# tomwhite/disq

Measured on AMD Instinct MI355X. Metric: decompressed BAM GB/s + reads/sec (whole node) at 1/2/4/8 MI355X, higher is better.
Workload: dtype u8

## Files before the change

### disq_amd/csrc/dq_api.hip

```cpp
#include <hip/hip_runtime.h>

#include <fcntl.h>
#include <sys/stat.h>
#include <unistd.h>

#include <algorithm>
#include <chrono>
#include <cstdio>
#include <cstdlib>
#include <cstring>
#include <map>
#include <string>
#include <thread>
#include <type_traits>
#include <sys/mman.h>
#include <mutex>
#include <vector>

#include "../../include/disq_gpu.h"
#include "dq_internal.h"
#include "dq_sam_core.h"
#include "dq_vcf_core.h"
#include "dq_vcf_gt_core.h"
#include "dq_vcf_info_core.h"
// ... 647 lines not shown
  }
  dbg(s, "chain", nblk, broken);
  ctx->nblk = nblk;
  if (nblk == 0 && L > 0) RET(DQ_EFORMAT, "no BGZF blocks found");
  ctx->ulen = ulen;
  HIPCHK(hipEventRecord(ctx->ev[1], s));
  if ((rc = ensure_all(ctx, ctx->U, (size_t)ulen + 256))) return rc;
  if ((rc = ensure_all(ctx, ctx->status, sizeof(int32_t) * (size_t)(nblk + 1)))) return rc;
  HIPCHK(hipMemsetAsync(ctx->status.p, 0, sizeof(int32_t) * (size_t)(nblk + 1), s));
  HIPCHK(hipMemsetAsync(ctx->U.as<uint8_t>() + ulen, 0, 256, s));
  {
    const uint32_t* crc_init = inflate3_tables(ctx->o.device);
    if (!crc_init) RET(DQ_EDEVICE, "CRC32 table initialisation failed on this device");
    static const bool timing = getenv("DQ_TIMING") != nullptr;
    uint64_t* tim = nullptr;
    if (timing) {
      HIPCHK(hipMalloc(&tim, sizeof(uint64_t) * INFLATE_TIM_WORDS * (size_t)std::max<int64_t>(1, nblk)));
      HIPCHK(hipMemsetAsync(tim, 0, sizeof(uint64_t) * INFLATE_TIM_WORDS * (size_t)std::max<int64_t>(1, nblk), s));
    }
    HIPCHK(hipEventRecord(ctx->ev[5], s));
    if ((rc = ensure_all(ctx, ctx->tails, INFLATE_SCRATCH_BYTES * (size_t)std::max<int64_t>(1, nblk)))) return rc;
    launch_inflate3(ctx->cbuf(), ctx->blk_pos.as<int64_t>(), ctx->blk_cs.as<int32_t>(),
                    ctx->blk_us.as<int32_t>(), ctx->uoff.as<int64_t>(), nblk, ctx->U.as<uint8_t>(),
                    ctx->status.as<int32_t>(), ctx->o.verify_crc, crc_init, tim, s, nullptr, 0,
                    ctx->tails.p);
    HIPCHK(hipEventRecord(ctx->ev[6], s));
    if (timing) {
      std::vector<uint64_t> h(INFLATE_TIM_WORDS * (size_t)nblk);
      HIPCHK(hipMemcpyAsync(h.data(), tim, 8 * h.size(), hipMemcpyDeviceToHost, s));
      HIPCHK(hipStreamSynchronize(s));
      (void)hipFree(tim);
      double acc[24] = {0};
      for (int64_t i = 0; i < nblk; i++)
        for (int k = 0; k < 24; k++) acc[k] += (double)h[32 * (size_t)i + k];
      static const char* nm[16] = {"header", "tables", "spec", "rounds", "scan", "emit",
                                   "resolve+store", "crc", "hdr_read_lengths", "resolve_hop_next", "redo_rounds", "tables_build",
                                   "resolve_steps_jumps", "resolve_store", "resolve_jump_tail", "res_batches"};
      fprintf(stderr, "[dq] inflate3 phase cycles per BGZF block (thread 0, s_memtime):");
      for (int k = 0; k < 16; k++)
        if (nm[k][0] != '-') fprintf(stderr, " %s=%.0f", nm[k], acc[k] / (double)std::max<int64_t>(1, nblk));
      fprintf(stderr, "\n");
      const double nb = (double)std::max<int64_t>(1, nblk);
      fprintf(stderr, "[dq] first deflate block: header=%.0f tables=%.0f spec=%.0f rounds=%.0f emit=%.0f; "
              "later ones: header=%.0f tables=%.0f spec=%.0f rounds=%.0f emit=%.0f; deflate blocks per "
              "BGZF block %.3f\n", acc[16] / nb, acc[17] / nb, acc[18] / nb, acc[19] / nb, acc[21] / nb,
              (acc[0] - acc[16]) / nb, (acc[1] - acc[17]) / nb, (acc[2] - acc[18]) / nb,
              (acc[3] - acc[19]) / nb, (acc[5] - acc[21]) / nb, acc[22] / nb);
      double rr[7] = {0};
      for (int64_t i = 0; i < nblk; i++)
        for (int k = 0; k < 7; k++) rr[k] += (double)h[32 * (size_t)i + 24 + k];
      fprintf(stderr, "[dq] rounds' re-decodes per BGZF block: lanes=%.2f merged=%.2f (mean checkpoint %.2f) "
              "unmerged: spec err/eob=%.2f spec exit=%.2f other=%.2f\n", rr[0] / nb, rr[2] / nb,
              rr[3] / std::max(1.0, rr[2]), rr[4] / nb, rr[5] / nb, rr[6] / nb);
      double ta[16] = {0};
      for (int64_t i = 0; i < nblk; i++)
        for (int k = 0; k < 16; k++) ta[k] += (double)h[32 * (size_t)nblk + 16 * (size_t)i + k];
      if (ta[3] > 0)
        fprintf(stderr, "[dq] tail kernel: %.0f tails (%.1f %% of blocks), cycles per tail (lane 0): "
                "decode=%.0f (header=%.0f tables=%.0f spec=%.0f rounds=%.0f emit=%.0f) "
                "rows=%.0f store_crc=%.0f\n", ta[3], 100.0 * ta[3] / nb, ta[0] / ta[3],
                ta[4] / ta[3], ta[5] / ta[3], ta[6] / ta[3], ta[7] / ta[3], ta[8] / ta[3],
                ta[1] / ta[3], ta[2] / ta[3]);
      if (ta[3] > 0)
        fprintf(stderr, "[dq] tail rows per tail %.1f, jump rounds per row %.2f, rows with in-row chains %.1f %%, "
                "round cycles per tail %.0f\n", ta[9] / ta[3], ta[10] / std::max(1.0, ta[9]),
                100.0 * ta[11] / std::max(1.0, ta[9]), ta[12] / ta[3]);
      for (int tl = 0; tl < 2; tl++) {
        double hp[8] = {0};
        const int64_t nw = (nblk + 63) / 64;
        for (int64_t w = 0; w < nw; w++)
          for (int k = 0; k < 8; k++) hp[k] += (double)h[48 * (size_t)nblk + 8 * (size_t)(2 * w + tl) + k];
        if (hp[5] > 0)
          fprintf(stderr, "[dq] header pre-pass (%s): %.0f waves, cycles per wave (lane 0): loads=%.0f "
                  "cl_code=%.0f cl_table=%.0f lengths=%.0f write=%.0f\n", tl ? "tails" : "first blocks",
                  hp[5], hp[0] / hp[5], hp[1] / hp[5], hp[2] / hp[5], hp[3] / hp[5], hp[4] / hp[5]);
      }
    }
  }
  dbg(s, "inflate", nblk, ulen);
  HIPCHK(hipEventRecord(ctx->ev[2], s));
  unsigned long long* d_bad = reinterpret_cast<unsigned long long*>(ctx->scal.as<char>() + 144);
  const bool defer_bad = ctx->shard && !ctx->header_only && !ctx->text_mode;
  unsigned long long bad = ~0ull;
  HIPCHK(hipMemsetAsync(d_bad, 0xff, 8, s));
  launch_first_bad(ctx->status.as<int32_t>(), nullptr, nblk, d_bad, s);
  auto bad_block = [&]() -> int {
    int32_t st = 0;
    int64_t pos = 0;
    HIPCHK(hipMemcpy(&st, ctx->status.as<int32_t>() + bad, 4, hipMemcpyDeviceToHost));
    HIPCHK(hipMemcpy(&pos, ctx->blk_pos.as<int64_t>() + bad, 8, hipMemcpyDeviceToHost));
    char msg[256];
    snprintf(msg, sizeof msg, "%s in BGZF block at %lld", status_name(st), (long long)pos);
    RET(DQ_EFORMAT, msg);
  };
  if (!defer_bad) {
    HIPCHK(hipMemcpyAsync(&bad, d_bad, 8, hipMemcpyDeviceToHost, s));
    HIPCHK(hipStreamSynchronize(s));
    if (bad != ~0ull) return bad_block();
  }
  if (ctx->text_mode) {
    ctx->stats = dq_stats{};
    ctx->stats.ms_scan = ev_ms(ctx->ev[0], ctx->ev[1]);
    ctx->stats.ms_inflate = ev_ms(ctx->ev[5], ctx->ev[6]);
    ctx->have_pipeline = true;
    return 0;
  }
// ... 3903 lines not shown
```

### disq_amd/csrc/dq_inflate3.hip

```cpp
#include "dq_hdr_core.h"
#include "dq_inflate_core.h"
#include "dq_internal.h"

#include <mutex>
#include <vector>

namespace dq {
namespace {

using namespace dqi;

#define DQ_HD __device__ __host__ __attribute__((always_inline)) inline

#ifndef DQ_BLK_WG
#define DQ_BLK_WG 512
#endif
constexpr int WG = DQ_BLK_WG;
static_assert(WG % 128 == 0 && WG >= 512 && WG <= 1024, "whole waves on every SIMD");
constexpr int NWV = WG / 64;
constexpr int NDEC = WG;
constexpr uint32_t OV_DEFAULT = 96;
#ifndef DQ_TAIL_OV
#define DQ_TAIL_OV OV_DEFAULT
#endif
// ... 296 lines not shown
  DQ_CHK(LT::kLSUB + (e >> 7) + ((bb >> LR) & ((1u << sb) - 1)) < (uint32_t)LT::kDROOT, CHK_K2_TABLE);
  if (!SLOW) return L.u.d.T[LT::kLSUB + (e >> 7) + ((bb >> LR) & ((1u << sb) - 1))];
  if (sb) return L.u.d.T[LT::kLSUB + (e >> 7) + ((bb >> LR) & ((1u << sb) - 1))];
  if (!(e & E_SLOW)) return 0u;
  int l = 0;
  const int k = canon_decode(bb, L.u.d.hl, LR + 1, &l);
  return k < 0 ? 0u : L.u.d.lent[k];
}
template <bool SLOW, class LT>
DQ_AI uint32_t d_second(const LT& L, uint32_t e, uint32_t bb) {
  const uint32_t sb = (e >> 4) & 7;
  DQ_CHK(LT::kDSUB + (e >> 7) + ((bb >> DR) & ((1u << sb) - 1)) < (uint32_t)LT::kTEND, CHK_K2_TABLE);
  if (!SLOW) return L.u.d.T[LT::kDSUB + (e >> 7) + ((bb >> DR) & ((1u << sb) - 1))];
  if (sb) return L.u.d.T[LT::kDSUB + (e >> 7) + ((bb >> DR) & ((1u << sb) - 1))];
  if (!(e & E_SLOW)) return 0u;
  int l = 0;
  const int k = canon_decode(bb, L.u.d.hd, DR + 1, &l);
  return k < 0 ? 0u : L.u.d.dent[k];
}


template <bool SLOW, class S, class LT>
DQ_AI bool dsym(BitR& r, const S& W, const LT& L, uint32_t p, uint32_t lim,
                uint32_t& len, uint32_t& dist, uint32_t& lit2, bool& is_m, uint32_t& e) {
  br_refill(r, W);
  uint32_t bb = br_peek(r);
  const uint32_t ri = bb & ((1u << LR) - 1);
  e = L.u.d.T[ri];
  uint32_t pe = 0;
  if constexpr (LT::kPair) pe = zx16(L.u.d.x.pair[ri]);
  if ((e & 15) == 0) e = ll_second<SLOW>(L, e, bb);
  const uint32_t nb = e & 15;
  const uint32_t lx = __builtin_amdgcn_ubfe(e, 5, 3);
  is_m = (e & 16) != 0;
  len = (e >> 8) + (is_m ? 3u : 0u) + __builtin_amdgcn_ubfe(bb, nb, lx);
  const bool two = pe != 0 && p + nb < lim;
  lit2 = two ? pe >> 8 : 0xffffffffu;
  br_take(r, W, nb + lx + (two ? (pe & 15) : 0u));
  br_refill(r, W);
  bb = br_peek(r);
  uint32_t e2 = zx16(L.u.d.T[LT::kDROOT + (bb & ((1u << DR) - 1))]);
  if (is_m && (e2 & 15) == 0) e2 = d_second<SLOW>(L, e2, bb);
  const uint32_t nb2 = e2 & 15, dx = __builtin_amdgcn_ubfe(e2, 4, 4);
  dist = (__builtin_amdgcn_ubfe(e2, 12, 2) << __builtin_amdgcn_ubfe(e2, 8, 4)) + 1u +
         __builtin_amdgcn_ubfe(bb, nb2, dx);
  br_take(r, W, is_m ? nb2 + dx : 0u);
  return (SLOW && nb == 0) || (e & 0xFEF0u) == 0xF810u ||
         (is_m && ((SLOW && nb2 == 0) || (e2 & 0x4000u)));
}
DQ_AI uint32_t stop_end(uint32_t e, uint32_t p) {
  return (e & 15) != 0 && (e & 0xFFF0u) == LL_EOB ? p + (e & 15) : 0xffffffffu;
}

enum : int32_t { F_DEAD = 4 };

constexpr int NCK_DEFAULT = 8;
constexpr uint32_t CKI_DEFAULT = 48;

template <bool SLOW, class S, class LT>
DQ_AI int run_seg(const S& W, const LT& L, uint32_t start, uint32_t sB,
                  uint32_t sE, uint32_t endbits, int32_t* Bp, int32_t* Ep, int32_t* cntp,
                  uint32_t* ck, int ckstride, uint32_t CKI, int NCK) {
  BitR r;
  br_init(r, W, start);
  uint32_t p = br_pos(r);
  uint32_t len = 0, dist = 0, lit2, e = 0;
  bool m;
  const uint32_t sBe = min(sB, endbits);
  while (p < sBe) {
    if (dsym<SLOW>(r, W, L, p, sBe, len, dist, lit2, m, e)) {
      len = stop_end(e, p);
      *Ep = (int32_t)(len != 0xffffffffu ? len : p);
      *Bp = -1;
      *cntp = 0;
      return F_DEAD;
    }
    p = br_pos(r);
  }
  if (p < sB) {
    *Ep = (int32_t)p;
    *Bp = -1;
    *cntp = 0;
    return F_DEAD;
  }
  const int32_t B = (int32_t)p;
  int32_t cnt = 0;
  int f;
  uint32_t thr = ck ? sB + CKI : 0xffffffffu;
  uint32_t* const dummy = const_cast<uint32_t*>(L.scratch) + (tid_fresh() & 15);
  uint32_t* ckp = ck;
  const uint32_t* const cke = ck + NCK * ckstride;
  const uint32_t sEe = min(sE, endbits);
  bool stopped;
  for (;;) {
    const bool cross = p >= thr;
    const bool st = cross && ckp < cke;
    *(st ? ckp : dummy) = ((p - sB) << 16) | (uint32_t)cnt;
    ckp += st ? ckstride : 0;
    thr += cross ? CKI : 0u;
    stopped = false;
    if (p >= sEe) break;
    stopped = true;
    if (dsym<SLOW>(r, W, L, p, min(thr, sEe), len, dist, lit2, m, e)) break;
    cnt += m ? (int32_t)len : (lit2 != 0xffffffffu ? 2 : 1);
    p = br_pos(r);
  }
  if (stopped) {
    len = stop_end(e, p);
    *Ep = (int32_t)(len != 0xffffffffu ? len : p);
    f = len != 0xffffffffu ? F_EOB : F_ERR;
  } else {
    *Ep = (int32_t)p;
    f = p >= sE ? F_EXIT : F_END;
  }
  *Bp = B;
  *cntp = cnt;
  return f;
}

template <bool SLOW, class S, class LT>
DQ_AI int run_redo(const S& W, const LT& L, uint32_t s0, uint32_t sB,
                   uint32_t sE, uint32_t endbits, const uint32_t* ck, int ckstride, int32_t se,
                   int32_t sc, int32_t* Ep, int32_t* cntp, uint32_t CKI, int NCK, int* jm = nullptr) {
  BitR r;
  br_init(r, W, s0);
  int32_t cnt = 0;
  int f;
  uint32_t thr = ck ? sB + CKI : 0xffffffffu;
  uint32_t cur = ck ? ck[0] : 0xffffffffu;
  const uint32_t* ckq = ck;
  const uint32_t* const ckl = ck + (NCK - 1) * ckstride;
  const uint32_t sEe = min(sE, endbits);
  int j = 0;
  int why;
  uint32_t p, len = 0, e = 0;
  for (;;) {
    p = br_pos(r);
    const bool cross = p >= thr;
    const bool merge = cross && (cur >> 16) == p - sB;
    why = merge ? 1 : 0;
    if (p >= sEe || merge) break;
    const bool more = ckq < ckl;
    if (jm) j += cross ? 1 : 0;
    ckq += cross && more ? ckstride : 0;
    const uint32_t nxt = ck ? *ckq : 0xffffffffu;
    thr += cross ? CKI : 0u;
    cur = cross ? (more ? nxt : 0xffffffffu) : cur;
    uint32_t dist = 0, lit2;
    bool m;
    why = 2;
    if (dsym<SLOW>(r, W, L, p, min(thr, sEe), len, dist, lit2, m, e)) break;
    cnt += m ? (int32_t)len : (lit2 != 0xffffffffu ? 2 : 1);
  }
  if (why == 1) {
    *Ep = se >> 3;
    f = se & 7;
    cnt += sc - (int32_t)(cur & 0xffffu);
    if (jm) *jm = j;
  } else if (why == 2) {
    len = stop_end(e, p);
    *Ep = (int32_t)(len != 0xffffffffu ? len : p);
    f = len != 0xffffffffu ? F_EOB : F_ERR;
  } else {
    *Ep = (int32_t)p;
    f = p >= sE ? F_EXIT : F_END;
  }
  *cntp = cnt;
  return f;
}

template <bool SLOW, class S, class LT>
DQ_AI void emit_seg(const S& W, LT& L, uint32_t start, uint32_t target,
                    uint32_t endbits, int32_t p, int32_t isize, int sh, int32_t ibase = 0) {
  typedef volatile __attribute__((address_space(3))) uint8_t lds8;
  uint32_t* const dummy32 = emit_dummy(L) + (tid_fresh() & 63);
  lds8* const dummy1 = (lds8*)dummy32 - 1;
  lds8* const dummy2 = (lds8*)dummy32 - 2;
  BitR r;
  br_init(r, W, start);
  const uint32_t te = min(target, endbits);
  int32_t obase = sh - ibase;
  asm("" : "+v"(obase));
  bool bad = false;
  for (;;) {
    const uint32_t q = br_pos(r);
    if (q >= te || p >= isize) break;
    uint32_t len = 0, dist = 0, lit2;
    bool m;
    uint32_t e;
    const bool stop = dsym<SLOW>(r, W, L, q, te, len, dist, lit2, m, e);
    const bool far = m && (int32_t)dist > p;
    bad = far && !stop;
    if (stop || far) break;
    const bool two = !m && lit2 != 0xffffffffu && p + 1 < isize;
    DQ_CHK(p >= ibase && sh + p - ibase + 2 < (int)sizeof(L.out) &&
               ((p - ibase) >> 5) < (int)(sizeof(L.bm) / 4), CHK_K2_IMAGE);
    const uint32_t desc = (dist - 1) | ((len - 3) << 15);
    lds8* const o = (lds8*)(L.out + (obase + p));
    o[0] = (uint8_t)(m ? desc : len);
    (m || two ? o : dummy1)[1] = (uint8_t)(m ? desc >> 8 : lit2);
    (m ? o : dummy2)[2] = (uint8_t)(desc >> 16);
    atomicOr(m ? &L.bm[(p - ibase) >> 5] : dummy32, 1u << ((p - ibase) & 31));
    p += m ? (int32_t)len : (two ? 2 : 1);
  }
  if (bad) set_err(L, ST_BAD_DIST);
}

__device__ inline uint32_t gf2_mulmod(uint32_t a, uint32_t b) {
  uint32_t p = 0;
#pragma unroll
  for (int i = 31; i >= 0; i--) {
    p ^= ((a >> i) & 1u) ? b : 0u;
    b = (b >> 1) ^ ((b & 1u) ? 0xEDB88320u : 0u);
  }
  return p;
}

DQ_AI int wave_incl_scan(int v, int) {
  v += __builtin_amdgcn_update_dpp(0, v, 0x111, 0xf, 0xf, false);
  v += __builtin_amdgcn_update_dpp(0, v, 0x112, 0xf, 0xf, false);
  v += __builtin_amdgcn_update_dpp(0, v, 0x114, 0xf, 0xf, false);
  v += __builtin_amdgcn_update_dpp(0, v, 0x118, 0xf, 0xf, false);
  v += __builtin_amdgcn_update_dpp(0, v, 0x142, 0xa, 0xf, false);
  v += __builtin_amdgcn_update_dpp(0, v, 0x143, 0xc, 0xf, false);
  return v;
}
DQ_AI int wave_incl_or(int v) {
  v |= __builtin_amdgcn_update_dpp(0, v, 0x111, 0xf, 0xf, false);
  v |= __builtin_amdgcn_update_dpp(0, v, 0x112, 0xf, 0xf, false);
  v |= __builtin_amdgcn_update_dpp(0, v, 0x114, 0xf, 0xf, false);
  v |= __builtin_amdgcn_update_dpp(0, v, 0x118, 0xf, 0xf, false);
  v |= __builtin_amdgcn_update_dpp(0, v, 0x142, 0xa, 0xf, false);
  v |= __builtin_amdgcn_update_dpp(0, v, 0x143, 0xc, 0xf, false);
  return v;
}
DQ_AI uint32_t wave_incl_xor(uint32_t v) {
  v ^= (uint32_t)__builtin_amdgcn_update_dpp(0, (int)v, 0x111, 0xf, 0xf, false);
// ... 332 lines not shown
    take[1] = onp[1] && have_w + rinc[1] - rp[1] < total;
    int val[2];
    val[0] = (take[0] && s[0] == 16) ? (key0 > 0 ? (key0 & 31) : prev_w) : v00;
    val[1] = (take[1] && s[1] == 16) ? (key1 > 0 ? (key1 & 31) : prev_w) : v01;
    if ((take[0] && (adv[0] == 0 || (s[0] == 16 && val[0] < 0))) ||
        (take[1] && (adv[1] == 0 || (s[1] == 16 && val[1] < 0))))
      set_err(L, ST_BAD_TABLE);
#pragma unroll
    for (int h = 0; h < 2; h++) {
      const int r = take[h] ? rep[h] : 0;
      if (take[h] && val[h] != 0) {
        for (int i = have_w + rinc[h] - r; i < have_w + rinc[h] && i < total; i++)
          H.lens[i < nlen ? i : 288 + i - nlen] = (uint8_t)val[h];
      }
    }
    if (have_w < total && have_w + H.wt[w] >= total) {
      const uint64_t mark0 = __ballot(take[0]), mark1 = __ballot(take[1]);
      const int lastl = mark1 ? 64 + 63 - __clzll(mark1) : 63 - __clzll(mark0);
      const int ll = lastl & 63;
      const int cum = have_w + (lastl >= 64 ? __builtin_amdgcn_readlane(rinc[1], ll) : __builtin_amdgcn_readlane(rinc[0], ll));
      const int j = lastl + (lastl >= 64 ? __builtin_amdgcn_readlane(adv[1], ll) : __builtin_amdgcn_readlane(adv[0], ll));
      if (lane == 0) {
        if (cum > total) set_err(L, ST_BAD_TABLE);
        H.endp = (int32_t)(Wb + (uint32_t)j);
      }
    }
    have += wsum;
    prev = lvall;
    const uint32_t nextP = P + 128u * NWV + (uint32_t)H.ent[NWV];
    if (have < total && H.ent[NWV] >= 16) {
      set_err(L, ST_BAD_TABLE);
      return P;
    }
    __syncthreads();
    if (L.misc[M_ERR]) return P;
    P = nextP;
  }
  if (have < total) {
    set_err(L, ST_BAD_TABLE);
    return P;
  }
  return (uint32_t)H.endp;
}

template <bool TIMING, int NB, int G>
__global__ __launch_bounds__(WG, WG / 128) void inflate_block_kernel(
    const uint8_t* __restrict__ C, const int64_t* __restrict__ blk_pos,
    const int32_t* __restrict__ blk_csize, const int32_t* __restrict__ blk_usize,
    const int64_t* __restrict__ uoff, int64_t nblk, uint8_t* __restrict__ U,
    int32_t* __restrict__ status, int32_t verify_crc, const uint32_t* __restrict__ crc_init,
    uint64_t* __restrict__ tim, uint32_t OV, uint32_t sflags, const int32_t* __restrict__ sel,
    TailDesc* __restrict__ tails) {
  constexpr uint32_t CKI = CKI_DEFAULT;
  constexpr int NCK = NCK_DEFAULT;
  __shared__ LdsI L;
  uint64_t tacc[24] = {0, 0, 0, 0, 0, 0, 0, 0, 0, 0, 0, 0, 0, 0, 0, 0, 0, 0, 0, 0, 0, 0, 0, 0};
  uint64_t tlast = TIMING ? __builtin_amdgcn_s_memtime() : 0;
#define TST(i)                                            \
  do {                                                    \
    if (TIMING && threadIdx.x == 0) {                     \
      const uint64_t now_ = __builtin_amdgcn_s_memtime(); \
      tacc[i] += now_ - tlast;                            \
      tlast = now_;                                       \
    }                                                     \
  } while (0)
#define TCOUNT(i) do { if (TIMING && threadIdx.x == 0) tacc[i] += 1; } while (0)
  if ((int64_t)blockIdx.x >= nblk) return;
  const int64_t b = sel ? (int64_t)sel[blockIdx.x] : (int64_t)blockIdx.x;
  const int t = threadIdx.x, lane = t & 63, wv = t >> 6;
  const int64_t cpos = blk_pos[b];
  const int32_t csize = blk_csize[b];
  const int32_t isize = blk_usize[b];
  const int64_t ub = uoff[b];
  const int sh = (int)(ub & 15);
  const uint8_t* dp = C + cpos + 18;
  const int mis = (int)(reinterpret_cast<uintptr_t>(dp) & 15);
  const uint32_t* W =
      reinterpret_cast<const uint32_t*>(__builtin_assume_aligned(dp - mis, 16));
  const uint32_t a0 = 8u * (uint32_t)mis;
  const int32_t dbytes = csize - 26;
  const uint32_t endbits = a0 + 8u * (uint32_t)max(dbytes, 0);

  uint32_t warm = 0;
  if ((sflags & 16) && 128u * (uint32_t)t < (uint32_t)(mis + max(dbytes, 0))) warm = W[32 * t];
  const bool hon = (sflags & 32) != 0;
  uint32_t hinfo = 0;
  if (hon) {
    const HdrMeta* hrec = reinterpret_cast<const HdrMeta*>(tails + nblk);
    const HdrMeta* hm = hrec + blockIdx.x + (tid_fresh() >> 10);
    hinfo = hm->info;
    if (hm_kind(hinfo) == dqh::HDR_DYN && t < HDR_LW) {
      const uint32_t w = reinterpret_cast<const uint32_t*>(hrec + nblk)[(int64_t)blockIdx.x * HDR_LW + t];
      uint32_t* l8 = reinterpret_cast<uint32_t*>(L.u.d.x.h.lens);
      l8[2 * t] = nib4(w & 0xffffu);
      l8[2 * t + 1] = nib4(w >> 16);
    }
    if (t == M_A) L.misc[M_A] = (int32_t)hm->end;
    if (t == M_HDR) L.misc[M_HDR] = hm_kind(hinfo) == dqh::HDR_DYN ? (int32_t)hinfo : 0;
  }
  for (int i = t; i < 2048; i += WG) L.bm[i] = 0;
  if (t < 32 && !(hon && (t == M_A || t == M_HDR))) L.misc[t] = 0;
  if (t == 0) {
    if (isize < 0 || isize > 65536) L.misc[M_ERR] = ST_ISIZE;
    else if (dbytes < 0) L.misc[M_ERR] = ST_OVERREAD;
    else if (isize > 0 && hm_kind(hinfo) == dqh::HDR_ERR) L.misc[M_ERR] = hm_status(hinfo);
  }
  asm volatile("" ::"v"(warm));
  __syncthreads();
  int32_t produced = 0;
  uint32_t pos = a0;
  bool deferred = false;
  while (L.misc[M_ERR] == 0 && produced < isize) {
    const int t = tid_fresh(), lane = t & 63, wv = t >> 6;
    if (t == 0) L.misc[M_SLOW] = 0;
    const uint32_t clpos = pos + 17;
    const uint32_t hbase = clpos >> 5;
    const bool hpre = L.misc[M_HDR] != 0;
    const uint32_t hw = !hpre && t < HB_WORDS ? W[hbase + t] : 0u;
    const uint32_t hcl = !hpre && t < 19 ? peek_bits(W, clpos + 3 * t, 3) : 0u;
    const uint32_t h = peek_bits(W, pos, 17);
    const int32_t bfinal = (int32_t)(h & 1), btype = (int32_t)((h >> 1) & 3);
    const int32_t herr = pos + 3 > endbits ? ST_OVERREAD : btype == 3 ? ST_BAD_BLOCKTYPE : 0;
// ... 74 lines not shown
          v = (uint16_t)e2;
      }
      L.u.d.x.pair[i] = v;
    }
    __syncthreads();
    TST(1);
    const uint32_t a = (uint32_t)L.misc[M_A];
    const bool slow = L.misc[M_SLOW] != 0;
    if (a > endbits) {
      if (t == 0) L.misc[M_ERR] = ST_OVERREAD;
      break;
    }
    const uint32_t span = endbits - a;
    const int ob = (sh + produced + 3) & ~3;
    const int cap = (sh + isize - ob) / (4 * (7 + NCK));
    int32_t* AB;
    int32_t* AE;
    int32_t* AC;
    int32_t* LS;
    int32_t* ST;
    int32_t* SE;
    int32_t* SC;
    uint32_t* CK = nullptr;
    const uint32_t maxl = (sflags >> 8) & 1023u, minseg = (sflags >> 20) & 1023u;
    int nl = (int)max(1u, min(maxl ? maxl : (uint32_t)NDEC, span / (minseg ? minseg : 128u)));
    nl = cap >= 8 ? min(nl, cap) : min(nl, 8);
    const uint32_t seg = (span + nl - 1) / nl;
    if (seg) nl = (int)((span + seg - 1) / seg);
    AB = cap >= 8 ? reinterpret_cast<int32_t*>(L.out + ob) : L.small;
    AE = AB + nl;
    AC = AE + nl;
    LS = AC + nl;
    ST = LS + nl;
    SE = ST + nl;
    SC = SE + nl;
    if (cap >= 8) CK = reinterpret_cast<uint32_t*>(SC + nl);
    DQ_CHK(cap < 8 || (ob >= sh + produced && ob + 4 * nl * (7 + NCK) <= OUTCAP), CHK_K2_LANES);
#ifdef DQ_CHECKED
    GSrc gsrc{W, (endbits >> 5) + 8, 1u << 12};
#else
    const GSrc gsrc{W};
#endif
    if (t == 0) {
      L.misc[M_RCNT] = 0;
      L.misc[M_LAST] = nl - 1;
    }
    if (t < nl) {
      const uint32_t sB = a + (uint32_t)t * seg;
      const uint32_t start = t == 0 ? a : (sB > a + OV ? sB - OV : a);
      const uint32_t sE = t == nl - 1 ? 0xffffffffu : a + (uint32_t)(t + 1) * seg;
      int32_t B = -1, E = 0, c = 0;
      if (CK)
        for (int j = 0; j < NCK; j++) CK[j * nl + t] = 0xffffffffu;
      const int f = slow ? run_seg<true>(gsrc, L, start, sB, sE, endbits, &B, &E, &c,
                                         CK ? CK + t : nullptr, nl, CKI, NCK)
                         : run_seg<false>(gsrc, L, start, sB, sE, endbits, &B, &E, &c,
                                          CK ? CK + t : nullptr, nl, CKI, NCK);
      AB[t] = B;
      AE[t] = (E << 3) | f;
      AC[t] = c;
      SE[t] = (E << 3) | f;
      SC[t] = c;
    }
    __syncthreads();
    TST(2);
#ifdef DQ_CHECKED
    gsrc.tag = 2u << 12;
#endif
    for (int round = 0; round <= nl; round++) {
      bool need = false;
      int32_t st = 0;
      if (t > 0 && t < nl) {
        const int32_t pe = AE[t - 1];
        st = pe >> 3;
        need = (pe & 7) == F_EXIT && AB[t] != st;
      }
      int32_t* rc = &L.misc[M_RCNT + (round & 1)];
      if (need) {
        const int r = atomicAdd(rc, 1);
        DQ_CHK(r < nl, CHK_K2_LANES);
        LS[r] = t;
        ST[r] = st;
      }
      if (t == 0) {
        L.misc[M_RCNT + ((round + 1) & 1)] = 0;
        L.misc[M_DIRTY + (round & 1)] = 0;
      }
      __syncthreads();
      const int nneed = *rc;
      if (nneed == 0) break;
      TCOUNT(10);
      const bool hi = __builtin_amdgcn_readfirstlane(t) < __builtin_amdgcn_readfirstlane(nneed);
      if (hi) __builtin_amdgcn_s_setprio(3);
      if (t < nneed) {
        const int lt = LS[t];
        const uint32_t s0 = (uint32_t)ST[t];
        const uint32_t sE = lt == nl - 1 ? 0xffffffffu : a + (uint32_t)(lt + 1) * seg;
        int32_t E = 0, c = 0;
        int jmerge = -1;
        const uint32_t sB = a + (uint32_t)lt * seg;
        const int f = slow ? run_redo<true>(gsrc, L, s0, sB, sE, endbits, CK ? CK + lt : nullptr,
                                            nl, SE[lt], SC[lt], &E, &c, CKI, NCK,
                                            TIMING ? &jmerge : nullptr)
                           : run_redo<false>(gsrc, L, s0, sB, sE, endbits, CK ? CK + lt : nullptr,
                                             nl, SE[lt], SC[lt], &E, &c, CKI, NCK,
                                             TIMING ? &jmerge : nullptr);
        const int32_t ae = (E << 3) | f;
        if (ae != AE[lt]) L.misc[M_DIRTY + (round & 1)] = 1;
        AB[lt] = (int32_t)s0;
        AE[lt] = ae;
        AC[lt] = c;
        if (TIMING) {
          atomicAdd(&L.misc[21], 1);
          if (jmerge >= 0) {
            atomicAdd(&L.misc[23], 1);
            atomicAdd(&L.misc[24], jmerge);
          } else {
            const int sf = SE[lt] & 7;
            atomicAdd(&L.misc[sf == F_ERR || sf == F_EOB ? 25 : sf == F_EXIT ? 26 : 27], 1);
          }
        }
      }
      if (hi) __builtin_amdgcn_s_setprio(0);
      __syncthreads();
      if (L.misc[M_DIRTY + (round & 1)] == 0) break;
    }
    TST(3);

    int32_t myB = 0, myE = 0, myF = F_DEAD, myC = 0;
    if (t < nl) {
      myB = AB[t];
      myE = AE[t] >> 3;
      myF = AE[t] & 7;
      myC = AC[t];
    }
    if (t < nl && myF != F_EXIT) atomicMin(&L.misc[M_LAST], t);
    __syncthreads();
    const int last = L.misc[M_LAST];
    const int32_t cv = t <= last ? myC : 0;
    const int32_t incl = wave_incl_scan(cv, lane);
    if (lane == 63) L.wsum[wv] = incl;
    if (t == last) {
      L.misc[M_NEXT] = myE;
      L.misc[M_LASTF] = myF;
    }
    __syncthreads();
    int32_t woff = 0;
    for (int w = 0; w < wv; w++) woff += L.wsum[w];
    const int32_t myoff = produced + woff + incl - cv;
    int32_t total = 0;
    for (int w = 0; w < WG / 64; w++) total += L.wsum[w];
    const bool full = produced + total >= isize;
    const int32_t fl = L.misc[M_LASTF];
    if (!full && fl != F_EOB && t == 0) L.misc[M_ERR] = fl == F_ERR ? ST_BAD_CODE : ST_SHORT;
    __syncthreads();
    TST(4);
    if (L.misc[M_ERR]) break;
#ifdef DQ_CHECKED
    gsrc.tag = 3u << 12;
#endif
    if (t <= last && myoff < isize) {
      const uint32_t sE = t == nl - 1 ? 0xffffffffu : a + (uint32_t)(t + 1) * seg;
      if (slow) emit_seg<true>(gsrc, L, (uint32_t)myB, sE, endbits, myoff, isize, sh);
      else emit_seg<false>(gsrc, L, (uint32_t)myB, sE, endbits, myoff, isize, sh);
    }
    const int32_t nextpos = L.misc[M_NEXT];
    __syncthreads();
    TST(5);
    produced = min(isize, produced + total);
    if (TIMING && t == 0) {
      if (tacc[22] == 0)
        for (int i = 0; i < 6; i++) tacc[16 + i] = tacc[i];
      tacc[22] += 1;
    }
    if (full || bfinal) break;
    pos = (uint32_t)nextpos;
    if (tails && isize - produced <= TOUT && endbits - pos <= (uint32_t)TAIL_MAX_BITS) {
      deferred = true;
      break;
    }
  }
  __syncthreads();
  int32_t err = L.misc[M_ERR];
  if (!err && !deferred && produced != isize) err = ST_SHORT;
  const int32_t rsize = deferred ? produced : isize;
  if (deferred && t == 0) {
    TailDesc td;
    td.pos = (int32_t)pos;
    td.produced = produced;
    td.crc_raw = 0;
    td.flag = 1;
    tails[blockIdx.x] = td;
  }
  if (err) {
    if (t == 0) status[b] = err;
    return;
  }
  const uint64_t* bm64 = reinterpret_cast<const uint64_t*>(L.bm);
  {
    int ls[2];
    int run = -1;
#pragma unroll
    for (int k = 0; k < 2; k++) {
      const uint64_t m = 2 * t + k < 1024 ? bm64[min(2 * t + k, 1023)] : 0ull;
      if (m) run = 64 * (2 * t + k) + 63 - __clzll(m);
      ls[k] = run;
    }
    const int wm = wave_incl_max(run);
    if (lane == 63) L.wsum[wv] = wm;
    int ex = __shfl_up(wm, 1, 64);
    if (lane == 0) ex = -1;
    __syncthreads();
    for (int w = 0; w < wv; w++) ex = max(ex, L.wsum[w]);
#pragma unroll
    for (int k = 0; k < 2; k++) {
      const int v = max(ex, ls[k]);
      if (WG == 512 || 2 * t + k < 1024) L.u.r.last_start[2 * t + k] = v < 0 ? (uint16_t)0xffff : (uint16_t)v;
    }
    __syncthreads();
  }
  uint8_t* dstU = U + ub;
  const uint8_t* O = L.out + sh;
  const int head = min((16 - sh) & 15, rsize);
  int32_t lines_done = 0;
  constexpr int CH = G * WG;
  constexpr int BATCH = NB * CH;
  constexpr int NE = NB * G;
  constexpr bool CSTEP = (DQ_CSTEP != 0 && G > 1) || CH % 512 != 0;
  static_assert(BATCH <= RES_NXT, "the batch's next-pointers fit the resolve scratch");
  static_assert((65536 + BATCH - 1) / BATCH <= NCARRY, "one carry slot per batch");
  static_assert(CSTEP || CH / 512 <= G, "the G ordered steps of a chunk cover it");
  constexpr bool QUAD = G == 4 && DQ_RES_QUAD != 0;
  constexpr bool HYB = G == 1 && NB == 4 && WG == 512 && !CSTEP && DQ_RES_QUAD != 0;
  constexpr int GK = HYB ? 1 : NB, GCH = HYB ? BATCH : CH;
  static_assert(!(QUAD || HYB) || offsetof(LdsI, u.r.nxt) % 8 == 0, "a group's next pointers are one 64-bit word");
// ... 324 lines not shown
  }
  uint32_t ct0 = 0, ct1 = 0, cshift = 0, cinit = 0, cwant = 0;
  if (verify_crc) {
    ct0 = (&c_crc4[0][0])[t];
    ct1 = t + WG < 1024 ? (&c_crc4[0][0])[t + WG] : 0u;
    cshift = c_slice_shift[WG - 1 - t];
    if (t == 0) {
      cinit = crc_init[rsize];
      const uint8_t* tr = C + cpos + csize - 8;
      cwant = (uint32_t)tr[0] | ((uint32_t)tr[1] << 8) | ((uint32_t)tr[2] << 16) | ((uint32_t)tr[3] << 24);
    }
  }
  static_assert(2 * WG >= 1024, "at most two CRC table words per thread");
  for (int x = t; x < head; x += WG) dstU[x] = O[x];
  for (int x = head + 16 * lines_done + t; x < rsize; x += WG) dstU[x] = O[x];
  TST(6);
  if (verify_crc) {
    __syncthreads();
    if (t < 1024) (&L.u.crc4[0][0])[t] = ct0;
    if (t + WG < 1024) (&L.u.crc4[0][0])[t + WG] = ct1;
    __syncthreads();
    const int32_t e = rsize - (WG - 1 - t) * CRC_SL;
    const int32_t s0 = max(0, e - CRC_SL);
    uint32_t cr = 0;
    if (e > 0) {
      int32_t x = s0;
      while (x < e && ((sh + x) & 3)) cr = L.u.crc4[0][(cr ^ O[x++]) & 0xff] ^ (cr >> 8);
      for (; x + 4 <= e; x += 4) {
        const uint32_t v = cr ^ *reinterpret_cast<const uint32_t*>(O + x);
        cr = L.u.crc4[3][v & 0xff] ^ L.u.crc4[2][(v >> 8) & 0xff] ^ L.u.crc4[1][(v >> 16) & 0xff] ^
             L.u.crc4[0][v >> 24];
      }
      while (x < e) cr = L.u.crc4[0][(cr ^ O[x++]) & 0xff] ^ (cr >> 8);
      cr = gf2_mulmod(cshift, cr);
    }
    cr = wave_incl_xor(cr);
    if (lane == 63) L.wsum[wv] = (int32_t)cr;
    __syncthreads();
    if (t == 0) {
      uint32_t x = 0;
      for (int w = 0; w < WG / 64; w++) x ^= (uint32_t)L.wsum[w];
      if (deferred) {
        tails[blockIdx.x].crc_raw = x;
      } else {
        const uint32_t crc = (x ^ cinit) ^ 0xffffffffu;
        if (crc != cwant) status[b] = ST_CRC;
      }
    }
  }
  TST(7);
  if (TIMING && t == 0)
    for (int i = 0; i < 24; i++) tim[(int64_t)blockIdx.x * TIM_W + i] = tacc[i];
  if (TIMING && t == 0)
    for (int i = 0; i < 7; i++) tim[(int64_t)blockIdx.x * TIM_W + 24 + i] = (uint64_t)L.misc[21 + i];
}

constexpr int HP_WIN = 16;
constexpr int HP_WAVES = 16;
struct HpSrc {
  const uint32_t* __restrict__ W;
  uint32_t last;
  uint32_t base;
  uint32_t w[HP_WIN];
  DQ_AI void load(uint32_t b0) {
    base = b0;
#pragma unroll
    for (int k = 0; k < HP_WIN; k++)
      w[k] = *reinterpret_cast<const uint32_t*>(reinterpret_cast<const uint8_t*>(W) + (min(b0 + (uint32_t)k, last) << 2));
  }
  DQ_AI void ahead(uint32_t i) {
    if (__any(i - base >= (uint32_t)(HP_WIN - 1))) load(i);
  }
  DQ_AI uint32_t word(uint32_t i) const {
    const uint32_t k = i - base;
    DQ_CHK(k < (uint32_t)HP_WIN, CHK_K2_BITS);
    uint32_t t[HP_WIN];
#pragma unroll
    for (int j = 0; j < HP_WIN; j++) t[j] = w[j];
#pragma unroll
    for (int h = HP_WIN / 2, bit = 1; h >= 1; h /= 2, bit *= 2)
#pragma unroll
      for (int j = 0; j < h; j++) t[j] = (k & (uint32_t)bit) ? t[2 * j + 1] : t[2 * j];
    return t[0];
  }
};
static_assert(HP_WIN >= 8 && (HP_WIN & (HP_WIN - 1)) == 0, "six words before the first ahead(); a tree of selects");
struct HpTbl {
  uint8_t* t;
  DQ_AI void set(uint32_t k, uint32_t v) { t[k * 64] = (uint8_t)v; }
  DQ_AI uint32_t get(uint32_t k) const { return t[k * 64]; }
};
template <bool TIMING>
struct HpSink {
  uint2* out;
  uint32_t cur;
  uint64_t acc;
  uint64_t c[4];
  uint64_t tm[3];
  DQ_AI void store() {
    DQ_CHK(cur < (uint32_t)(HDR_LW / 2), CHK_K2_LANES);
    out[cur] = make_uint2((uint32_t)acc, (uint32_t)(acc >> 32));
  }
  DQ_AI void run(uint32_t i, uint32_t n, uint32_t v) {
    const uint32_t u = i >> 4, p = i & 15;
    if (u != cur) {
      store();
      for (uint32_t k = cur + 1; k < u; k++) out[k] = make_uint2(0, 0);
// ... 902 lines not shown
```

### disq_amd/csrc/dq_internal.h

```cpp
#pragma once
#include <hip/hip_runtime.h>
#include <stdint.h>

enum : int32_t {
  ST_OK = 0,
  ST_BAD_HEADER = 1,
  ST_BAD_BLOCKTYPE = 2,
  ST_BAD_STORED = 3,
  ST_BAD_TABLE = 4,
  ST_BAD_CODE = 5,
  ST_BAD_DIST = 6,
  ST_SHORT = 7,
  ST_OVERREAD = 8,
  ST_CRC = 9,
  ST_ISIZE = 10,
  ST_HANG = 11,
  ST_TEXT_START = 12,
};

enum : int {
  CHK_K1_SLOT = 0,
  CHK_K2_BITS = 1,
  CHK_K2_IMAGE = 2,
  CHK_K2_TABLE = 3,
// ... 48 lines not shown
  z *= 0x94D049BB133111EBULL;
  z ^= z >> 31;
  return z;
}
#define DQ_K_LEN 0x9E3779B97F4A7C15ULL
#define DQ_K_WORD 0xD6E8FEB86659FD93ULL

namespace dq {

struct Cand {
  int64_t pos;
  int32_t csize;
  int32_t usize;
  int32_t valid;
  int32_t pad;
};

constexpr int SCAN_CHUNK = 16384;
constexpr int SCAN_CAP = 32;
constexpr int SCAN_CAP_BIG = 640;
constexpr int SCAN_OVER_MAX = 1 << 22;

void launch_bgzf_scan(const uint8_t* C, int64_t n, int64_t L, Cand* slots, int64_t cap,
                      int32_t* chunk_counts, int64_t n_chunks, int64_t* d_count,
                      int32_t* over_list, hipStream_t s);
void launch_bgzf_scan_listed(const uint8_t* C, int64_t n, int64_t L, Cand* big, int64_t n_over,
                             int32_t* chunk_counts, int32_t* over_list, int32_t* over_map,
                             hipStream_t s);
void launch_gather_slots(const Cand* slots, const int32_t* counts, const int64_t* offs,
                         int64_t nchunks, Cand* out, int64_t cap, const int32_t* over_map,
                         const Cand* big, hipStream_t s);
void launch_valid_flags(const Cand* cand, const int64_t* ncand, int64_t cap, int32_t* flags,
                        hipStream_t s);
void launch_chain2(const uint8_t* C, int64_t L, const Cand* cand, const int64_t* ncand, int64_t cap,
                   const int64_t* voff, int64_t* blk_pos, int32_t* blk_csize, int32_t* blk_usize,
                   int64_t blk_cap, int64_t* d_nblk, int32_t* d_broken, int32_t eof_in_buf,
                   hipStream_t s);
void launch_chain_check(const Cand* cand, const int64_t* d_ncand, int64_t cap, const int64_t* blk_pos,
                        const int64_t* d_nblk, unsigned long long* out, hipStream_t s);
void launch_first_bad(const int32_t* status, const int32_t* sel, int64_t n, unsigned long long* out,
                      hipStream_t s);
void launch_chain_serial(const uint8_t* C, int64_t clen, int64_t start, int64_t* blk_pos,
                         int32_t* blk_csize, int32_t* blk_usize, int64_t cap, int64_t* d_nblk,
                         int32_t* d_status, hipStream_t s);

void launch_exclusive_scan_i32(const int32_t* in, int64_t* out, int64_t n, int64_t* tmp,
                               hipStream_t s);
void launch_exclusive_scan_i64(const int64_t* in, int64_t* out, int64_t n, int64_t* tmp,
                               hipStream_t s);

const uint32_t* inflate3_tables(int device);
constexpr size_t INFLATE_SCRATCH_BYTES = 16 + (16 + 32) + 160;
constexpr size_t INFLATE_TIM_WORDS = 64;
void launch_inflate3(const uint8_t* C, const int64_t* blk_pos, const int32_t* blk_csize,
                     const int32_t* blk_usize, const int64_t* uoff, int64_t nblk, uint8_t* U,
                     int32_t* status, int32_t verify_crc, const uint32_t* crc_init, uint64_t* tim,
                     hipStream_t s, const int32_t* sel, int64_t nsel, void* scratch);

void launch_block_stats(const int64_t* blk_pos, const int32_t* blk_cs, const int64_t* uoff,
                        int64_t nblk, int64_t ulen, int64_t x, uint64_t* out, hipStream_t s);

constexpr int64_t SPLIT_FROM_SBI = -2;
struct SplitPlan {
  int64_t split_start, split_end;
  int64_t first_blk;
  int64_t u_lo, u_hi;
  int64_t rec_lin;
  uint64_t vstart, vend;
  int32_t status;
  int32_t rec_span;
};
void launch_plan_blocks(const Cand* cand, const int64_t* d_ncand, const int64_t* blk_pos,
                        const int32_t* blk_usize, const int64_t* uoff, const int64_t* d_nblk,
                        SplitPlan* plans, int64_t nsplit, hipStream_t s);
void launch_guess_all(const uint8_t* U, int64_t ulen, int32_t u_is_eof, const int32_t* ref_len,
                      int32_t n_ref, uint8_t* flag, hipStream_t s);
void launch_first_record(const uint8_t* U, int64_t ulen, int32_t u_is_eof, const int32_t* ref_len,
                         int32_t n_ref, const int64_t* blk_pos, const int64_t* uoff,
                         const int64_t* d_nblk, SplitPlan* plans, int64_t nsplit,
                         unsigned long long* best, hipStream_t s);

struct Seg {
  int64_t start;
  int64_t exit;
  int64_t count;
  int32_t exact;
  int32_t status;
};
constexpr int SEG_OFF_CAP = 512;
void launch_seg_spec(const uint8_t* U, int64_t ulen, int32_t u_is_eof, int64_t chain_end,
                     const int32_t* ref_len, int32_t n_ref, Seg* segs, int64_t nseg,
                     int64_t seg_bytes, int64_t start_lin, uint16_t* offs, hipStream_t s);
void launch_seg_link(const Seg* segs, int64_t nseg, int64_t seg_bytes, int64_t start_lin,
                     int64_t ulen, int32_t* d_broken, hipStream_t s);
void launch_seg_fix2(const uint8_t* U, int64_t ulen, int32_t u_is_eof, int64_t chain_end,
                     Seg* segs, int64_t nseg,
                     int64_t seg_bytes, int64_t start_lin, int32_t* d_status, hipStream_t s);
void launch_seg_counts(const Seg* segs, int64_t nseg, int64_t* counts, hipStream_t s);
void launch_seg_emit2(const uint8_t* U, int64_t ulen, const Seg* segs, const int64_t* base,
                      int64_t nseg, int64_t* rec_lin, hipStream_t s, const uint16_t* offs = nullptr,
                      int64_t seg_bytes = 0, int64_t start_lin = 0);

struct Win {
  int64_t u_start;
  int64_t u_chain_end;
  int64_t u_limit;
// ... 270 lines not shown
```

Before: 200.9.

## Split speculative and redo decode loops into checkpoint and plain phases, record three checkpoints

The speculative segment decode and the redo decode loops are each split into two phases. The first phase records or merges against checkpoints. Once the last checkpoint is passed, the wave switches (by ballot vote) to a lean loop with no checkpoint bookkeeping. The default number of recorded checkpoints drops from eight to three, which cuts stores and merge comparisons but leaves fewer chances to merge early in redo rounds. It also re-derives the thread id after the decode phase to ease register pressure, and adds a per-checkpoint merge histogram to the timing output.

```diff
diff --git a/disq_amd/csrc/dq_api.hip b/disq_amd/csrc/dq_api.hip
--- a/disq_amd/csrc/dq_api.hip
+++ b/disq_amd/csrc/dq_api.hip
@@ -723,6 +723,13 @@
       fprintf(stderr, "[dq] rounds' re-decodes per BGZF block: lanes=%.2f merged=%.2f (mean checkpoint %.2f) "
               "unmerged: spec err/eob=%.2f spec exit=%.2f other=%.2f\n", rr[0] / nb, rr[2] / nb,
               rr[3] / std::max(1.0, rr[2]), rr[4] / nb, rr[5] / nb, rr[6] / nb);
+      double mh[8] = {0};
+      for (int64_t i = 0; i < nblk; i++)
+        for (int k = 0; k < 8; k++)
+          mh[k] += (double)((h[32 * (size_t)i + (k < 4 ? 25 : 31)] >> (16 * (k & 3))) & 0xffffu);
+      fprintf(stderr, "[dq] merges per BGZF block by checkpoint (%d recorded):", INFLATE_NCK_REC);
+      for (int k = 0; k < 8; k++) fprintf(stderr, " %d=%.2f", k, mh[k] / nb);
+      fprintf(stderr, "\n");
       double ta[16] = {0};
       for (int64_t i = 0; i < nblk; i++)
         for (int k = 0; k < 16; k++) ta[k] += (double)h[32 * (size_t)nblk + 16 * (size_t)i + k];
diff --git a/disq_amd/csrc/dq_inflate3.hip b/disq_amd/csrc/dq_inflate3.hip
--- a/disq_amd/csrc/dq_inflate3.hip
+++ b/disq_amd/csrc/dq_inflate3.hip
@@ -372,12 +372,29 @@
   return (e & 15) != 0 && (e & 0xFFF0u) == LL_EOB ? p + (e & 15) : 0xffffffffu;
 }
 
+#ifdef DQ_NO_LOOP_TAGS
+#define DQ_LOOP_TAG(name) do {} while (0)
+#else
+#define DQ_LOOP_TAG(name)                                  \
+  do {                                                     \
+    if (SLOW) asm volatile("; dq-loop " name " slow");     \
+    else asm volatile("; dq-loop " name);                  \
+  } while (0)
+#endif
+#ifndef DQ_SPLIT
+#define DQ_SPLIT 1
+#endif
+
 enum : int32_t { F_DEAD = 4 };
 
-constexpr int NCK_DEFAULT = 8;
+constexpr int NCK_REC = INFLATE_NCK_REC;
+static_assert(NCK_REC >= 1 && NCK_REC <= 8, "the DQ_TIMING merge histogram has eight bins");
 constexpr uint32_t CKI_DEFAULT = 48;
 
-template <bool SLOW, class S, class LT>
+#ifndef DQ_HEAD_VOTE
+#define DQ_HEAD_VOTE 1
+#endif
+template <bool SLOW, bool SPLIT = false, class S, class LT>
 DQ_AI int run_seg(const S& W, const LT& L, uint32_t start, uint32_t sB,
                   uint32_t sE, uint32_t endbits, int32_t* Bp, int32_t* Ep, int32_t* cntp,
                   uint32_t* ck, int ckstride, uint32_t CKI, int NCK) {
@@ -388,6 +405,7 @@
   bool m;
   const uint32_t sBe = min(sB, endbits);
   while (p < sBe) {
+    DQ_LOOP_TAG("warm-up");
     if (dsym<SLOW>(r, W, L, p, sBe, len, dist, lit2, m, e)) {
       len = stop_end(e, p);
       *Ep = (int32_t)(len != 0xffffffffu ? len : p);
@@ -410,20 +428,34 @@
   uint32_t* const dummy = const_cast<uint32_t*>(L.scratch) + (tid_fresh() & 15);
   uint32_t* ckp = ck;
   const uint32_t* const cke = ck + NCK * ckstride;
+  const uint32_t thl = ck ? sB + CKI * (uint32_t)NCK : 0u;
   const uint32_t sEe = min(sE, endbits);
   bool stopped;
   for (;;) {
+    DQ_LOOP_TAG("spec-head");
     const bool cross = p >= thr;
-    const bool st = cross && ckp < cke;
+    const bool st = cross && (SPLIT ? thr <= thl : ckp < cke);
     *(st ? ckp : dummy) = ((p - sB) << 16) | (uint32_t)cnt;
     ckp += st ? ckstride : 0;
     thr += cross ? CKI : 0u;
     stopped = false;
     if (p >= sEe) break;
+    if (SPLIT && (DQ_HEAD_VOTE ? __builtin_amdgcn_ballot_w64(thr <= thl) == 0 : thr > thl)) break;
     stopped = true;
     if (dsym<SLOW>(r, W, L, p, min(thr, sEe), len, dist, lit2, m, e)) break;
     cnt += m ? (int32_t)len : (lit2 != 0xffffffffu ? 2 : 1);
     p = br_pos(r);
+  }
+  if (SPLIT && !stopped) {
+    for (;;) {
+      DQ_LOOP_TAG("spec-tail");
+      stopped = false;
+      if (p >= sEe) break;
+      stopped = true;
+      if (dsym<SLOW>(r, W, L, p, sEe, len, dist, lit2, m, e)) break;
+      cnt += m ? (int32_t)len : (lit2 != 0xffffffffu ? 2 : 1);
+      p = br_pos(r);
+    }
   }
   if (stopped) {
     len = stop_end(e, p);
@@ -438,7 +470,7 @@
   return f;
 }
 
-template <bool SLOW, class S, class LT>
+template <bool SLOW, bool SPLIT = false, class S, class LT>
 DQ_AI int run_redo(const S& W, const LT& L, uint32_t s0, uint32_t sB,
                    uint32_t sE, uint32_t endbits, const uint32_t* ck, int ckstride, int32_t se,
                    int32_t sc, int32_t* Ep, int32_t* cntp, uint32_t CKI, int NCK, int* jm = nullptr) {
@@ -454,7 +486,44 @@
   int j = 0;
   int why;
   uint32_t p, len = 0, e = 0;
-  for (;;) {
+  if constexpr (SPLIT) {
+    why = 3;
+    if (ck) {
+      for (;;) {
+        DQ_LOOP_TAG("redo-merge");
+        p = br_pos(r);
+        const bool cross = p >= thr;
+        const bool merge = cross && (cur >> 16) == p - sB;
+        const bool last = cross && ckq >= ckl;
+        why = merge ? 1 : last ? 3 : 0;
+        if (p >= sEe || merge || last) break;
+        if (jm) j += cross ? 1 : 0;
+        ckq += cross ? ckstride : 0;
+        const uint32_t nxt = *ckq;
+        thr += cross ? CKI : 0u;
+        cur = cross ? nxt : cur;
+        uint32_t dist = 0, lit2;
+        bool m;
+        why = 2;
+        if (dsym<SLOW>(r, W, L, p, min(thr, sEe), len, dist, lit2, m, e)) break;
+        cnt += m ? (int32_t)len : (lit2 != 0xffffffffu ? 2 : 1);
+      }
+    }
+    if (why == 3) {
+      for (;;) {
+        DQ_LOOP_TAG("redo-plain");
+        p = br_pos(r);
+        why = 0;
+        if (p >= sEe) break;
+        uint32_t dist = 0, lit2;
+        bool m;
+        why = 2;
+        if (dsym<SLOW>(r, W, L, p, sEe, len, dist, lit2, m, e)) break;
+        cnt += m ? (int32_t)len : (lit2 != 0xffffffffu ? 2 : 1);
+      }
+    }
+  } else for (;;) {
+    DQ_LOOP_TAG("redo-merge");
     p = br_pos(r);
     const bool cross = p >= thr;
     const bool merge = cross && (cur >> 16) == p - sB;
@@ -501,8 +570,10 @@
   const uint32_t te = min(target, endbits);
   int32_t obase = sh - ibase;
   asm("" : "+v"(obase));
+  asm("" : "+v"(isize));
   bool bad = false;
   for (;;) {
+    DQ_LOOP_TAG("emit");
     const uint32_t q = br_pos(r);
     if (q >= te || p >= isize) break;
     uint32_t len = 0, dist = 0, lit2;
@@ -941,7 +1012,7 @@
     uint64_t* __restrict__ tim, uint32_t OV, uint32_t sflags, const int32_t* __restrict__ sel,
     TailDesc* __restrict__ tails) {
   constexpr uint32_t CKI = CKI_DEFAULT;
-  constexpr int NCK = NCK_DEFAULT;
+  constexpr int NCK = NCK_REC;
   __shared__ LdsI L;
   uint64_t tacc[24] = {0, 0, 0, 0, 0, 0, 0, 0, 0, 0, 0, 0, 0, 0, 0, 0, 0, 0, 0, 0, 0, 0, 0, 0};
   uint64_t tlast = TIMING ? __builtin_amdgcn_s_memtime() : 0;
@@ -956,7 +1027,7 @@
 #define TCOUNT(i) do { if (TIMING && threadIdx.x == 0) tacc[i] += 1; } while (0)
   if ((int64_t)blockIdx.x >= nblk) return;
   const int64_t b = sel ? (int64_t)sel[blockIdx.x] : (int64_t)blockIdx.x;
-  const int t = threadIdx.x, lane = t & 63, wv = t >> 6;
+  int t = threadIdx.x, lane = t & 63, wv = t >> 6;
   const int64_t cpos = blk_pos[b];
   const int32_t csize = blk_csize[b];
   const int32_t isize = blk_usize[b];
@@ -1137,10 +1208,10 @@
       int32_t B = -1, E = 0, c = 0;
       if (CK)
         for (int j = 0; j < NCK; j++) CK[j * nl + t] = 0xffffffffu;
-      const int f = slow ? run_seg<true>(gsrc, L, start, sB, sE, endbits, &B, &E, &c,
-                                         CK ? CK + t : nullptr, nl, CKI, NCK)
-                         : run_seg<false>(gsrc, L, start, sB, sE, endbits, &B, &E, &c,
-                                          CK ? CK + t : nullptr, nl, CKI, NCK);
+      const int f = slow ? run_seg<true, DQ_SPLIT != 0>(gsrc, L, start, sB, sE, endbits, &B, &E, &c,
+                                               CK ? CK + t : nullptr, nl, CKI, NCK)
+                         : run_seg<false, DQ_SPLIT != 0>(gsrc, L, start, sB, sE, endbits, &B, &E, &c,
+                                                CK ? CK + t : nullptr, nl, CKI, NCK);
       AB[t] = B;
       AE[t] = (E << 3) | f;
       AC[t] = c;
@@ -1184,12 +1255,12 @@
         int32_t E = 0, c = 0;
         int jmerge = -1;
         const uint32_t sB = a + (uint32_t)lt * seg;
-        const int f = slow ? run_redo<true>(gsrc, L, s0, sB, sE, endbits, CK ? CK + lt : nullptr,
-                                            nl, SE[lt], SC[lt], &E, &c, CKI, NCK,
-                                            TIMING ? &jmerge : nullptr)
-                           : run_redo<false>(gsrc, L, s0, sB, sE, endbits, CK ? CK + lt : nullptr,
-                                             nl, SE[lt], SC[lt], &E, &c, CKI, NCK,
-                                             TIMING ? &jmerge : nullptr);
+        const int f = slow ? run_redo<true, DQ_SPLIT != 0>(gsrc, L, s0, sB, sE, endbits, CK ? CK + lt : nullptr,
+                                                  nl, SE[lt], SC[lt], &E, &c, CKI, NCK,
+                                                  TIMING ? &jmerge : nullptr)
+                           : run_redo<false, DQ_SPLIT != 0>(gsrc, L, s0, sB, sE, endbits, CK ? CK + lt : nullptr,
+                                                   nl, SE[lt], SC[lt], &E, &c, CKI, NCK,
+                                                   TIMING ? &jmerge : nullptr);
         const int32_t ae = (E << 3) | f;
         if (ae != AE[lt]) L.misc[M_DIRTY + (round & 1)] = 1;
         AB[lt] = (int32_t)s0;
@@ -1200,6 +1271,9 @@
           if (jmerge >= 0) {
             atomicAdd(&L.misc[23], 1);
             atomicAdd(&L.misc[24], jmerge);
+            atomicAdd(reinterpret_cast<unsigned long long*>(tim + (int64_t)blockIdx.x * TIM_W +
+                                                            (jmerge < 4 ? 25 : 31)),
+                      1ull << (16 * (jmerge & 3)));
           } else {
             const int sf = SE[lt] & 7;
             atomicAdd(&L.misc[sf == F_ERR || sf == F_EOB ? 25 : sf == F_EXIT ? 26 : 27], 1);
@@ -1266,6 +1340,9 @@
     }
   }
   __syncthreads();
+  t = tid_fresh();
+  __builtin_assume((unsigned)t < (unsigned)WG);
+  lane = t & 63, wv = t >> 6;
   int32_t err = L.misc[M_ERR];
   if (!err && !deferred && produced != isize) err = ST_SHORT;
   const int32_t rsize = deferred ? produced : isize;
@@ -1696,7 +1773,8 @@
   if (TIMING && t == 0)
     for (int i = 0; i < 24; i++) tim[(int64_t)blockIdx.x * TIM_W + i] = tacc[i];
   if (TIMING && t == 0)
-    for (int i = 0; i < 7; i++) tim[(int64_t)blockIdx.x * TIM_W + 24 + i] = (uint64_t)L.misc[21 + i];
+    for (int i = 0; i < 7; i++)
+      if (i != 1) tim[(int64_t)blockIdx.x * TIM_W + 24 + i] = (uint64_t)L.misc[21 + i];
 }
 
 constexpr int HP_WIN = 16;
diff --git a/disq_amd/csrc/dq_internal.h b/disq_amd/csrc/dq_internal.h
--- a/disq_amd/csrc/dq_internal.h
+++ b/disq_amd/csrc/dq_internal.h
@@ -124,6 +124,10 @@
 const uint32_t* inflate3_tables(int device);
 constexpr size_t INFLATE_SCRATCH_BYTES = 16 + (16 + 32) + 160;
 constexpr size_t INFLATE_TIM_WORDS = 64;
+#ifndef DQ_NCK_REC
+#define DQ_NCK_REC 3
+#endif
+constexpr int INFLATE_NCK_REC = DQ_NCK_REC;
 void launch_inflate3(const uint8_t* C, const int64_t* blk_pos, const int32_t* blk_csize,
                      const int32_t* blk_usize, const int64_t* uoff, int64_t nblk, uint8_t* U,
                      int32_t* status, int32_t verify_crc, const uint32_t* crc_init, uint64_t* tim,
```

Result: no change. 200.4 (-0.2%).
